# quantumgizmos/bp_osd

Hardware: AMD Instinct MI355X
Metric: syndromes decoded/sec (whole node) + logical error rate, HGP [[1922,50]] p=0.05 (higher is better)
Workload: dtype f64; 1 GPU; h1922_ms_cs7: [[1922,50]] HGP (31x31 circulant 1+x^2+x^5) hz 961x1922, min-sum BP variable scaling, max_iter=1922, osd_cs order 7, iid bit-flip q=0.05; per_gpu_batch=131072, global_batch=131072, bp_variant=0, pipelined_steps=2, hw_queues=4, batches=2 distinct seeded batches alternate over the timed steps

## Files before the change

### bp_osd_amd/_lib.py

```python
from __future__ import annotations

import ctypes as C
import os

_HERE = os.path.dirname(os.path.abspath(__file__))
LIB_PATH = os.environ.get("BPOSD_LIB") or os.path.join(_HERE, "libbposd_mi355x.so")

BPOSD_OK = 0
BPOSD_ERR_INVALID = -1
BPOSD_ERR_UNSUPPORTED = -2
BPOSD_ERR_HIP = -3
BPOSD_ERR_NO_DEVICE = -4

EXPORTED_SYMBOLS = (
    "bposd_device_count",
    "bposd_version",
    "bposd_create",
    "bposd_update_channel_probs",
    "bposd_decode_batch",
    "bposd_decode_batch_packed",
    "bposd_decode_batch_async",
    "bposd_decode_batch_packed_async",
    "bposd_decode_batch_device",
    "bposd_decode_batch_device_packed",
# ... 9 lines not shown
    "bposd_host_alloc",
    "bposd_host_free",
    "bposd_last_timing",
    "bposd_info",
    "bposd_posterior_llr",
    "bposd_set_bp_variant",
    "bposd_set_osd_variant",
    "bposd_last_osd_kernel",
    "bposd_mc_create",
    "bposd_mc_run",
    "bposd_mc_fetch",
    "bposd_mc_device_bytes",
    "bposd_mc_last_error",
    "bposd_mc_destroy",
    "bposd_last_error",
    "bposd_destroy",
)

DEBUG_SYMBOLS = (
    "bposd_layout_info",
    "bposd_bp_kernel_info",
    "bposd_debug_local_layout",
    "bposd_debug_local_keys",
    "bposd_debug_class_layout",
    "bposd_debug_last_instance",
)


class BposdConfig(C.Structure):
    _fields_ = [
        ("device", C.c_int32),
        ("bp_method", C.c_int32),
        ("ms_scaling_factor", C.c_double),
        ("max_iter", C.c_int32),
        ("osd_method", C.c_int32),
        ("osd_order", C.c_int32),
        ("sort_tie_policy", C.c_int32),
        ("weight_fn", C.c_int32),
        ("schedule", C.c_int32),
        ("ps_clip", C.c_double),
        ("osd_e_bit_order", C.c_int32),
        ("ps_math_form", C.c_int32),
    ]


class BposdMcConfig(C.Structure):
# ... 61 lines not shown
    lib.bposd_lane_timing.restype = C.c_int
    lib.bposd_host_alloc.argtypes = [C.c_size_t]
    lib.bposd_host_alloc.restype = vp
    lib.bposd_host_free.argtypes = [vp]
    lib.bposd_host_free.restype = None
    lib.bposd_last_timing.argtypes = [vp, C.POINTER(C.c_double), C.POINTER(C.c_double),
                                      C.POINTER(C.c_int64), C.POINTER(C.c_int64)]
    lib.bposd_last_timing.restype = C.c_int
    lib.bposd_info.argtypes = [vp, C.POINTER(C.c_int32), C.POINTER(C.c_int32), C.POINTER(C.c_int32),
                               C.POINTER(C.c_int32)]
    lib.bposd_info.restype = C.c_int
    lib.bposd_layout_info.argtypes = [vp, C.POINTER(C.c_int64), C.POINTER(C.c_int64), C.POINTER(C.c_int64)]
    lib.bposd_layout_info.restype = C.c_int
    lib.bposd_pack_rows_device_lane.argtypes = [vp, C.c_int32, vp, C.c_int64, C.c_int32, vp]
    lib.bposd_pack_rows_device_lane.restype = C.c_int
    lib.bposd_posterior_llr.argtypes = [vp, vp, C.c_int64, vp, vp, vp, vp]
    lib.bposd_posterior_llr.restype = C.c_int
    lib.bposd_bp_kernel_info.argtypes = [vp, C.POINTER(C.c_int32), vp]
    lib.bposd_bp_kernel_info.restype = C.c_int
    lib.bposd_debug_local_layout.argtypes = [vp, vp, C.c_int32, C.c_int32, vp]
    lib.bposd_debug_local_layout.restype = C.c_int
    lib.bposd_debug_local_keys.argtypes = [vp, vp, C.c_int32, C.c_int32, vp, vp, vp]
    lib.bposd_debug_local_keys.restype = C.c_int
    lib.bposd_debug_class_layout.argtypes = [vp, vp, C.c_int32, C.c_int32, vp, vp, vp, vp, vp, vp]
    lib.bposd_debug_class_layout.restype = C.c_int
    lib.bposd_debug_last_instance.argtypes = [vp, vp, vp]
    lib.bposd_debug_last_instance.restype = C.c_int
    lib.bposd_set_osd_variant.argtypes = [vp, C.c_int32]
    lib.bposd_set_osd_variant.restype = C.c_int
    lib.bposd_last_osd_kernel.argtypes = [vp]
    lib.bposd_last_osd_kernel.restype = C.c_int
    lib.bposd_set_bp_variant.argtypes = [vp, C.c_int32]
    lib.bposd_set_bp_variant.restype = C.c_int
    lib.bposd_last_error.argtypes = [vp]
    lib.bposd_last_error.restype = C.c_char_p
    lib.bposd_destroy.argtypes = [vp]
    lib.bposd_destroy.restype = None
    lib.bposd_mc_create.argtypes = [C.POINTER(BposdMcConfig), vp, vp, vp, vp, C.c_int32, vp, vp, C.c_int32, C.c_int32, vp, vp, C.c_int32,
                                    vp, vp, vp, vp, C.POINTER(vp)]
    lib.bposd_mc_create.restype = C.c_int
    lib.bposd_mc_run.argtypes = [vp, C.c_uint64, C.c_int64, C.POINTER(C.c_int64)]
    lib.bposd_mc_run.restype = C.c_int
    lib.bposd_mc_fetch.argtypes = [vp, C.c_int32, vp, C.c_size_t]
    lib.bposd_mc_fetch.restype = C.c_int
    lib.bposd_mc_device_bytes.argtypes = [vp]
    lib.bposd_mc_device_bytes.restype = C.c_int64
# ... 27 lines not shown
```

### bp_osd_amd/csrc/bp_local_kernel.hip.h

```cpp
#pragma once
#include <hip/hip_runtime.h>
#include <stdint.h>

#include "bp_kernel.hip.h"
#include "local_keys.h"

#ifndef BPOSD_BPL_SIGN_ON_MAG
#define BPOSD_BPL_SIGN_ON_MAG 0
#endif
namespace bposd {

struct BpLocalParams {
    int m, n;
    long long B;
    int max_iter;
    double ms_scaling;
    int osd_enabled;
    int mp;
    const uint8_t* __restrict__ synd;
    const double* __restrict__ llr0;
    const uint8_t* __restrict__ sel;
    const double* __restrict__ llr0_alt;
    const int* __restrict__ pos_chk;
    const int* __restrict__ pos_bit;
// ... 58 lines not shown

__device__ __forceinline__ int bpl_table_load(const int* base, unsigned int lane_off, unsigned int const_off) {
    asm volatile("" : "+v"(lane_off));
    return *(const int*)((const char*)base + (lane_off + const_off));
}

static_assert(__is_trivially_copyable(BpLocalParams) && alignof(BpLocalParams) <= 8, "BpLocalParams is copied into the kernarg segment as it is");
typedef const __attribute__((address_space(4))) BpLocalParams* bpl_args_ptr;
__device__ __forceinline__ bpl_args_ptr bpl_args() {
    bpl_args_ptr a = (bpl_args_ptr)__builtin_amdgcn_kernarg_segment_ptr();
    asm volatile("" : "+s"(a));
    return a;
}

template <int V>
struct bpl_int {
    static constexpr int value = V;
};

__host__ __device__ constexpr bool bpl_specialised(int cpt, int mpt, int minw, bool early) {
    return !early && ((cpt == 1 && mpt == 1024 && minw == 8) || (cpt == 2 && mpt == 1024 && (minw == 8 || minw == 6)) || (cpt == 2 && mpt == 2048 && minw == 4));
}

template <int CPT, int MPT, int MINW, bool EARLY, bool UPRIOR, bool PACKED = false>
__global__ __launch_bounds__(MPT / CPT, MINW) void bp_local_kernel(const BpLocalParams P) {
    extern __shared__ __attribute__((aligned(16))) unsigned char smem[];
    const int m = P.m, n = P.n;
#ifdef BPOSD_DEBUG
    if (blockIdx.x == 0 && threadIdx.x == 0 && (bpl_args()->m != P.m || bpl_args()->counters != P.counters)) __builtin_trap();
#endif
    constexpr int NT = MPT / CPT;
    constexpr int MP = MPT;
    const int tid = threadIdx.x;
    const int lane = tid & 63;
    const int wave = __builtin_amdgcn_readfirstlane(tid >> 6);
    constexpr int NB = 2 * CPT;

    double* msg_plain = reinterpret_cast<double*>(smem);
    msg_ptr msg = (msg_ptr)msg_plain;
    unsigned int* diffw = reinterpret_cast<unsigned int*>(msg_plain + (size_t)4 * MP + 2);
    int* sh = reinterpret_cast<int*>(diffw + (MP / 32 + 2));
    const unsigned int diffw_base = (unsigned int)(uintptr_t)(__attribute__((address_space(3))) unsigned char*)diffw;

    typedef __attribute__((address_space(3))) unsigned char* lds_bytes;
    const unsigned int msg_base = (unsigned int)(uintptr_t)(lds_bytes)smem;
    unsigned int alo[NB], ahi[NB];
    int dl[NB];
    unsigned int dlpack = 0u;
    double l0[UPRIOR ? 1 : NB];
    if (UPRIOR) {
// ... 6 lines not shown
#pragma unroll
    for (int j = 0; j < CPT; ++j) {
        const int p = tid + j * NT;
#pragma unroll
        for (int b = 0; b < 2; ++b) {
            const int r = 2 * j + b;
            if (!UPRIOR) {
                const int bit = BPL_BIT(r);
                l0[r] = bit >= 0 ? bpl_args()->llr0[bit] : 1.0;
            }
            alo[r] = msg_base + 8u * (unsigned int)bpl_args()->pos_alo[b * MP + p];
            ahi[r] = msg_base + 8u * (unsigned int)bpl_args()->pos_ahi[b * MP + p];
            dl[r] = __builtin_amdgcn_readfirstlane(bpl_args()->grp_dl[b * (MP >> 6) + (p >> 6)]);
            dlpack |= (unsigned int)bpl_args()->pos_dl[b * MP + p] << (2 * r);
        }
    }

    int gkey[CPT];
#pragma unroll
    for (int j = 0; j < CPT; ++j) gkey[j] = bposd_local_keys::group_key(dl[2 * j], dl[2 * j + 1]);
    int wkey = gkey[0];
#pragma unroll
    for (int j = 1; j < CPT; ++j) wkey = (gkey[j] == wkey) ? wkey : -1;
    constexpr bool SPEC = bpl_specialised(CPT, MPT, MINW, EARLY);

    const int want_llr_s = __builtin_amdgcn_readfirstlane(bpl_args()->out_llr != nullptr ? 1 : 0);
    auto want_llr = [&]() -> bool {
        int w = want_llr_s;
        asm volatile("" : "+s"(w));
        return w != 0;
    };
    for (;;) {
        if (tid == 0) {
            int zero = 0;
            asm volatile("" : "+v"(zero));
            sh[0] = zero;
            sh[1] = zero;
            sh[2] = atomicAdd(&bpl_args()->counters[0], 1);
        }
        __syncthreads();
        const long long s = __builtin_amdgcn_readfirstlane(sh[2]);
        if (s >= P.B) {
            if (s == P.B && tid == 0 && bpl_args()->tail_flag) *(volatile int*)bpl_args()->tail_flag = 1;
            break;
        }

// ... 157 lines not shown
                        unsigned int pa = alo[r], pb = ahi[r];
                        asm volatile("" : "+v"(pa), "+v"(pb));
                        const int ca = (int)((pa - msg_base) >> 3) & (MP - 1), cb = (int)((pb - msg_base) >> 3) & (MP - 1);
                        const int co = tid + (r >> 1) * NT;
                        atomicXor(&diffw[ca >> 5], 1u << (ca & 31));
                        atomicXor(&diffw[cb >> 5], 1u << (cb & 31));
                        atomicXor(&diffw[co >> 5], 1u << (co & 31));
                    }
                };
                auto group_step = [&](const int j, auto gk_c) __attribute__((always_inline)) {
                    constexpr int GK = decltype(gk_c)::value;
                    bit_step(2 * j, bpl_int<bposd_local_keys::key_dl(GK, 0)>{});
                    bit_step(2 * j + 1, bpl_int<bposd_local_keys::key_dl(GK, 1)>{});
                };
#pragma unroll
                for (int j = 0; j < CPT; ++j) {
                    if ((2 * j) % BATCH == 0) {
#pragma unroll
                        for (int q = 2 * j; q < 2 * j + BATCH; ++q) {
                            X[q] = *BPL_AT(alo[q]);
                            Y[q] = *BPL_AT(ahi[q]);
                        }
                    }
                    if constexpr (KEY >= 0) group_step(j, bpl_int<KEY>{});
                    else {
                        switch (gkey[j]) {
                            case 0: group_step(j, bpl_int<0>{}); break;
                            case 1: group_step(j, bpl_int<1>{}); break;
                            case 2: group_step(j, bpl_int<2>{}); break;
                            case 5: group_step(j, bpl_int<5>{}); break;
                            case 6: group_step(j, bpl_int<6>{}); break;
                            case 10: group_step(j, bpl_int<10>{}); break;
                            default: group_step(j, bpl_int<bposd_local_keys::kMixedKey>{}); break;
                        }
                    }
                }
                __syncthreads();
            }
            return 0;
        };
        if (!conv) {
            int done = 0;
            int it_llr = 1;
            if (!want_llr()) {
                int wk = wkey;
                asm volatile("" : "+s"(wk));
                if constexpr (SPEC) {
                    switch (wk) {
                        case 0: done = iterate(bpl_int<0>{}, bpl_int<0>{}, 1); break;
                        case 1: done = iterate(bpl_int<1>{}, bpl_int<0>{}, 1); break;
                        case 2: done = iterate(bpl_int<2>{}, bpl_int<0>{}, 1); break;
                        case 5: done = iterate(bpl_int<5>{}, bpl_int<0>{}, 1); break;
                        case 6: done = iterate(bpl_int<6>{}, bpl_int<0>{}, 1); break;
                        case 10: done = iterate(bpl_int<10>{}, bpl_int<0>{}, 1); break;
                        case bposd_local_keys::kMixedKey: done = iterate(bpl_int<bposd_local_keys::kMixedKey>{}, bpl_int<0>{}, 1); break;
                        default: done = iterate(bpl_int<-1>{}, bpl_int<0>{}, 1); break;
                    }
                } else done = iterate(bpl_int<-1>{}, bpl_int<0>{}, 1);
                asm volatile("" : "+s"(done));
                it_llr = bpl_args()->max_iter;
                it_llr = it_llr > 1 ? it_llr : 1;
            }
            if (!done) iterate(bpl_int<-1>{}, bpl_int<1>{}, it_llr);
        }

        const bool to_osd = (!conv) && bpl_args()->osd_enabled;
        if (tid == 0) {
            if (to_osd) {
                const int slot = atomicAdd(&bpl_args()->counters[1], 1);
                bpl_args()->osd_list[slot] = (int)s;
                sh[3] = slot;
            }
            if (bpl_args()->out_conv) bpl_args()->out_conv[s] = conv ? 1 : 0;
            if (bpl_args()->out_iters) bpl_args()->out_iters[s] = it_done;
            if (it_done) atomicAdd(bpl_args()->iter_total, (unsigned long long)it_done);
        }
        __syncthreads();
        const int slot = to_osd ? sh[3] : 0;
        constexpr bool packed = PACKED;
// ... 32 lines not shown
```

### bp_osd_amd/csrc/bposd_capi.hip

```cpp
#include "../../include/bposd_mi355x.h"

#include <hip/hip_runtime.h>

#include <algorithm>
#include <cmath>
#include <cstdarg>
#include <cstdio>
#include <cstdlib>
#include <climits>
#include <cstring>
#include <string>
#include <tuple>
#include <functional>
#include <map>
#include <chrono>
#include <mutex>
#include <thread>
#include <vector>

#include "internal.h"
#include <array>
#include <vector>
#include <algorithm>
#include "local_layout.h"
// ... 282 lines not shown
    h->tab_dc = DC;
    h->tab_dv = DV;
    h->tab_mp = MP;
    h->tab_np = NP;
    return 0;
}
int build_tables_local(bposd_handle* h) {
    using namespace local_layout;
    h->local_ok = false;
    const int m = h->m, n = h->n;
    if (!(h->regular && h->dc_max == 6 && h->dv_max == 3 && n == 2 * m)) return 0;
    const int MP = m <= 1024 ? 1024 : 2048;
    if (m > MP) return 0;
    Graph g;
    Layout best;
    if (!local_layout_host(h->rp, h->ci, m, n, MP, g, best)) return 0;
    if (getenv("BPOSD_DEBUG_OCC"))
        fprintf(stderr, "[bposd] local-edge layout: bit pass %lld read cycles (floor %d) + %lld write cycles (floor %d), %d mixed pairs, %d uniform positions\n",
                best.passes, 4 * (MP / 32), best.wcycles, 6 * 4 * (MP / 64), best.mixed, best.nfull);
    h->local_passes = best.passes;
    h->local_wcycles = best.wcycles;

    const std::vector<int>&owner = best.owner, &load = best.load, &pos_of = best.pos_of, &pos_chk = best.pos_chk;
    const std::vector<int> grp_dl = group_dl_table(g, best);
    auto slot_of = [&](int c, int i) {
        int k = 0;
        for (int e = h->rp[c]; e < h->rp[c + 1]; ++e) {
            const int j = h->ci[e];
            if (owner[j] == c) continue;
            if (j == i) return k * MP + pos_of[c];
            ++k;
        }
        return -1;
    };
    std::vector<int> pos_bit(2 * (size_t)MP, -1), pos_alo(2 * (size_t)MP, 0), pos_ahi(2 * (size_t)MP, 0), pos_dl(2 * (size_t)MP, 0);
    for (int p = 0; p < MP; ++p)
        for (int b = 0; b < 2; ++b) {
            pos_alo[(size_t)b * MP + p] = (2 * b) * MP + p;
            pos_ahi[(size_t)b * MP + p] = (2 * b + 1) * MP + p;
        }
    for (int c = 0; c < m; ++c) {
        const int p = pos_of[c];
        for (int b = 0; b < 2; ++b) {
            const int i = load[2 * c + b];
            int o[2];
            g.others(i, c, o);
            const int sx = slot_of(o[0], i), sy = slot_of(o[1], i);
// ... 576 lines not shown

int bposd_bp_kernel_info(bposd_handle* h, int32_t* kernel, int64_t* lds_model) {
    if (!h) return BPOSD_ERR_INVALID;
    if (kernel) *kernel = h->last_bp_kernel;
    if (lds_model) {
        for (int k = 0; k < 4; ++k) lds_model[k] = 0;
        if (h->last_bp_kernel == BPOSD_BP_KERNEL_LOCAL) {
            lds_model[0] = h->local_passes; lds_model[1] = 4 * (h->local_mp / 32);
            lds_model[2] = h->local_wcycles; lds_model[3] = 6 * 4 * (h->local_mp / 64);
        } else if (h->last_bp_kernel == BPOSD_BP_KERNEL_CLASS) {
            lds_model[0] = h->class_read_cycles; lds_model[1] = h->class_read_floor;
            lds_model[2] = h->class_write_cycles; lds_model[3] = h->class_write_floor;
        } else if (h->last_bp_kernel == BPOSD_BP_KERNEL_LARGE) {
            lds_model[0] = h->large_form;
        }
    }
    return BPOSD_OK;
}

int bposd_debug_last_instance(bposd_handle* h, int32_t bp[6], int32_t osd[6]) {
    if (!h) return BPOSD_ERR_INVALID;
    if (bp) std::copy(h->last_bp_inst, h->last_bp_inst + 6, bp);
    if (osd) std::copy(h->last_osd_inst, h->last_osd_inst + 6, osd);
    return BPOSD_OK;
}

int bposd_synchronize(bposd_handle* h) {
    if (!h) return BPOSD_ERR_INVALID;
    DeviceGuard dev_guard(h->device);
    HIP_TRY(h, dev_guard.err);
    return sync_all_lanes(h);
}

static int decode_device_impl(bposd_handle* h, const uint8_t* d_synd, int64_t B, const uint8_t* d_sel,
                              uint8_t* d_osdw, uint8_t* d_osd0, uint8_t* d_bp, uint8_t* d_conv,
                              int32_t* d_iters, double* d_llr, int lane = -1, int rec_idx = 0, bool lean = false) {
    if (!h) return BPOSD_ERR_INVALID;
    if (B < 0 || B > 0x7fffffffLL) return fail(h, BPOSD_ERR_INVALID, "batch size %lld out of range", (long long)B);
    if (B == 0) return BPOSD_OK;
    if (!d_synd || !d_osdw) return fail(h, BPOSD_ERR_INVALID, "syndromes and osdw buffers are required");
    DeviceGuard dev_guard(h->device);
    HIP_TRY(h, dev_guard.err);
    if (lane < 0) {
        lane = h->next_lane;
        h->next_lane = (h->next_lane + 1) % h->nlanes;
        h->last_lane = lane;
// ... 681 lines not shown
        if (rp[c + 1] - rp[c] != 6) return BPOSD_ERR_UNSUPPORTED;
    std::vector<int> deg(n, 0);
    for (int e : ci) {
        if (e < 0 || e >= n) return BPOSD_ERR_INVALID;
        deg[e]++;
    }
    for (int i = 0; i < n; ++i)
        if (deg[i] != 3) return BPOSD_ERR_UNSUPPORTED;
    local_layout::Graph g;
    local_layout::Layout best;
    if (!local_layout_host(rp, ci, m, n, MP, g, best, false)) return BPOSD_ERR_UNSUPPORTED;
    local_layout::LdsCost t = local_layout::lds_cost(g, best);
    info[0] = t.read_cycles; info[1] = t.write_cycles; info[2] = t.mixed;
    if (local_layout::pair_groups(g, best) < 0) return BPOSD_ERR_UNSUPPORTED;
    t = local_layout::lds_cost(g, best);
    info[3] = t.read_cycles; info[4] = t.write_cycles; info[5] = t.mixed;
    info[6] = MP; info[7] = best.generic_waves;
    const std::vector<int> keys = local_layout::group_keys(g, best);
    for (int gq = 0; gq < MP / 64; ++gq) group_key[gq] = keys[gq];
    for (int p = 0; p < MP; ++p) pos_chk[p] = best.pos_chk[p];
    return BPOSD_OK;
}

int bposd_debug_class_layout(const int32_t* indptr, const int32_t* indices, int32_t m, int32_t n, int32_t* pos_chk, int32_t* pos_bit,
                             int32_t* bit_slot, int32_t* grp_deg, int32_t* grp_cdeg, int64_t* info) {
    if (!indptr || !indices || !info || m < 1 || n < 1) return BPOSD_ERR_INVALID;
    std::vector<int> rp(indptr, indptr + m + 1), ci(indices, indices + indptr[m]);
    for (int e : ci)
        if (e < 0 || e >= n) return BPOSD_ERR_INVALID;
    const ClassShape* shp = class_shape_for(rp, ci, m, n);
    if (!shp || m > 1024) return BPOSD_ERR_UNSUPPORTED;
    class_layout::Tables T;
    bool ok = false;
    for (int mp : {256, 512, 1024}) {
        if (m > mp) continue;
        if (class_layout::build(rp, ci, m, n, shp->dclo, shp->dc, shp->dvlo, shp->dvhi, kClassVPT, mp, mp, class_layout_iters(), T)) { ok = true; break; }
    }
    if (!ok) return BPOSD_ERR_UNSUPPORTED;
    info[0] = shp->dc; info[1] = shp->dvlo; info[2] = shp->dvhi; info[3] = kClassVPT; info[4] = T.MP; info[5] = T.NT;
    info[6] = T.read_cycles; info[7] = T.read_floor; info[8] = T.write_cycles; info[9] = T.write_floor; info[10] = shp->dclo;
    if (pos_chk) std::copy(T.pos_chk.begin(), T.pos_chk.end(), pos_chk);
    if (pos_bit) std::copy(T.pos_bit.begin(), T.pos_bit.end(), pos_bit);
    if (bit_slot) std::copy(T.bit_slot.begin(), T.bit_slot.end(), bit_slot);
    if (grp_deg) std::copy(T.grp_deg.begin(), T.grp_deg.end(), grp_deg);
    if (grp_cdeg) std::copy(T.grp_cdeg.begin(), T.grp_cdeg.end(), grp_cdeg);
    return BPOSD_OK;
// ... 14 lines not shown
```

### bp_osd_amd/csrc/internal.h

```cpp
#pragma once
#include "../../include/bposd_mi355x.h"
#include "../../include/bposd_mi355x_debug.h"

#include <hip/hip_runtime.h>

#include <algorithm>
#include <cstdio>
#include <cstdlib>
#include <string>
#include <vector>

#include "bp_kernel.hip.h"
#include "osd_kernel.hip.h"

struct DevBuf {
    void* p = nullptr;
    size_t bytes = 0;
};

constexpr int BPOSD_LANES = 4;
constexpr int BPOSD_MAX_CHUNKS = 16;

struct Lane {
    hipStream_t stream = nullptr;
// ... 51 lines not shown
    int dc_max = 0, dv_max = 0;
    bool regular = false;
    bool local_ok = false;
    int local_mp = 0;
    long long local_passes = 0;
    long long local_wcycles = 0;
    int *d_lpos_chk = nullptr, *d_lpos_bit = nullptr, *d_lpos_alo = nullptr, *d_lpos_ahi = nullptr, *d_lgrp_dl = nullptr, *d_lpos_dl = nullptr;
    bool bp_any = false;
    bool class_ok = false;
    int class_dclo = 0, class_dc = 0, class_dvlo = 0, class_dvhi = 0, class_mp = 0, class_nt = 0;
    long class_read_cycles = 0, class_write_cycles = 0, class_read_floor = 0, class_write_floor = 0;
    int *d_cpos_chk = nullptr, *d_cpos_bit = nullptr, *d_cbit_slot = nullptr, *d_cgrp_deg = nullptr, *d_cgrp_cdeg = nullptr;
    bool large = false;
    bool bp_hbm = false;
    int max_iter = 0;
    int rank = 0, kprime = 0, ncand = 0;
    bool probs_uniform = true;
    int bp_variant = 0;
    int last_bp_kernel = -1;
    int osd_variant = 0;
    int last_osd_kernel = -1;
    int32_t last_bp_inst[6] = {-1, 0, 0, 0, 0, 0};
    int32_t last_osd_inst[6] = {-1, 0, 0, 0, 0, 0};
    std::vector<int> rp, ci;
    std::vector<double> probs;
    int *d_rp = nullptr, *d_ci = nullptr;
    int *d_chk_deg = nullptr, *d_var_deg = nullptr, *d_var_pos = nullptr, *d_pos_bit = nullptr, *d_var_ck = nullptr;
    int large_form = 0;
    int tab_np = 0;
    long layout_cost = 0, layout_cost_natural = 0, layout_cost_ideal = 0;
    double* d_llr0 = nullptr;
    double* d_cost = nullptr;
    double *d_llr0_alt = nullptr, *d_cost_alt = nullptr;
    bool fp_weights = false;
    int *d_cp = nullptr, *d_ce = nullptr, *d_erow = nullptr, *d_lvl_ptr = nullptr, *d_lvl_bits = nullptr;
    int nlevels = 0;
    int tab_dc = 0, tab_dv = 0, tab_mp = 0;
    bool have_timing = false;
    long long batch_hint = 0;
    bool async_pending = false;
    hipStream_t osd_now = nullptr;
    uint8_t *cmp_osd0 = nullptr, *cmp_osdw = nullptr;
    bool bp_only = false;
    bool lane_alt = false;
    bool packed_now = false;
    bool tail_gate = false;
// ... 53 lines not shown
```

### bp_osd_amd/csrc/launch_bp_local.hip

```cpp
#include "internal.h"

#include "bp_local_kernel.hip.h"

using namespace bposd;
using namespace bposd_host;

namespace bposd_host {
template <int CPT, int MP, int MINW, bool EARLY, bool UPRIOR, bool PACKED>
static int launch_bp_local_tp(bposd_handle* h, const BpLocalParams& L);

template <int CPT, int MP, int MINW, bool EARLY, bool UPRIOR = false>
static int launch_bp_local_t(bposd_handle* h, const BpLocalParams& L) {
    constexpr bool has_packed = !EARLY && ((CPT == 1 && MP == 1024 && MINW == 8) || (CPT == 2 && MP == 1024 && (MINW == 8 || MINW == 6)) || MP == 2048);
    if constexpr (has_packed) {
        if (L.packed_io) return launch_bp_local_tp<CPT, MP, MINW, EARLY, UPRIOR, true>(h, L);
    } else {
        if (L.packed_io) return fail(h, BPOSD_ERR_UNSUPPORTED, "this BP kernel variant has no packed-I/O form");
    }
    return launch_bp_local_tp<CPT, MP, MINW, EARLY, UPRIOR, false>(h, L);
}

template <int CPT, int MP, int MINW, bool EARLY, bool UPRIOR, bool PACKED>
static int launch_bp_local_tp(bposd_handle* h, const BpLocalParams& L) {
    auto k = bp_local_kernel<CPT, MP, MINW, EARLY, UPRIOR, PACKED>;
    const int nt = MP / CPT;
    const size_t lds = bp_local_lds_bytes(L.mp);
    { int rc_lds = set_max_lds(h, (const void*)k, lds); if (rc_lds) return rc_lds; }
    int wg_per_cu = 1;
    { int rc_occ = cached_occupancy(h, (const void*)k, nt, lds, &wg_per_cu); if (rc_occ) return rc_occ; }
    if (getenv("BPOSD_DEBUG_OCC")) fprintf(stderr, "[bposd] local-edge BP kernel: %d threads, %zu B LDS, %d workgroups per CU\n", nt, lds, wg_per_cu);
    wg_per_cu = std::max(1, std::min(wg_per_cu, 8));
    long long grid = std::min<long long>(L.B, (long long)h->num_cu * wg_per_cu);
    if (grid < 1) grid = 1;
    int rc = ensure_lanes(h, &Lane::bpl_llr, sizeof(double) * (size_t)grid * h->n);
    if (rc) return rc;
    BpLocalParams Lq = L;
    Lq.llr_tmp = (double*)h->cur->bpl_llr.p;
    note_instance(h->last_bp_inst, BPOSD_BP_KERNEL_LOCAL, CPT, MP, MINW, EARLY, PACKED);
    hipLaunchKernelGGL(k, dim3((unsigned)grid), dim3(nt), lds, h->cur->stream, Lq);
    HIP_TRY(h, hipGetLastError());
    return 0;
}

int launch_bp_local(bposd_handle* h, const BpParams& P) {
    BpLocalParams L{};
    L.m = P.m; L.n = P.n; L.B = P.B; L.max_iter = P.max_iter; L.ms_scaling = P.ms_scaling; L.osd_enabled = P.osd_enabled;
    L.mp = h->local_mp;
    L.synd = P.synd; L.llr0 = P.llr0; L.sel = P.sel; L.llr0_alt = P.llr0_alt;
    L.pos_chk = h->d_lpos_chk; L.pos_bit = h->d_lpos_bit; L.pos_alo = h->d_lpos_alo; L.pos_ahi = h->d_lpos_ahi;
    L.grp_dl = h->d_lgrp_dl; L.pos_dl = h->d_lpos_dl;
    L.out_bp = P.out_bp; L.out_osd0 = P.out_osd0; L.out_osdw = P.out_osdw; L.out_conv = P.out_conv; L.out_iters = P.out_iters;
    L.out_llr = P.out_llr; L.llr_ws = P.llr_ws; L.osd_list = P.osd_list; L.counters = P.counters; L.iter_total = P.iter_total; L.tail_flag = P.tail_flag; L.packed_io = P.packed_io;
    if (h->local_mp == 2048) return launch_bp_local_t<2, 2048, 4, false>(h, L);
    if (h->bp_variant == 17) return launch_bp_local_t<2, 1024, 8, false>(h, L);
    if (h->bp_variant == 18) return launch_bp_local_t<1, 1024, 8, false>(h, L);
    if (h->bp_variant == 19) return launch_bp_local_t<4, 1024, 4, true>(h, L);
    if (h->bp_variant == 20) return launch_bp_local_t<2, 1024, 6, true>(h, L);
    if (h->bp_variant == 21) return launch_bp_local_t<4, 1024, 3, true>(h, L);
    const bool uprior = h->probs_uniform && !L.sel && h->probs[0] > 0.0 && h->probs[0] < 0.5;
    const long long work = h->batch_hint > 0 ? h->batch_hint : L.B;
    const bool small_call = h->bp_variant == 0 && work <= 40000;
    if (small_call) return uprior ? launch_bp_local_t<1, 1024, 8, false, true>(h, L) : launch_bp_local_t<1, 1024, 8, false>(h, L);
    if ((h->bp_variant == 22 || h->bp_variant == 0) && uprior) return launch_bp_local_t<2, 1024, 8, false, true>(h, L);
    if (h->bp_variant == 23 && uprior) return launch_bp_local_t<2, 1024, 6, true, true>(h, L);
    if (h->bp_variant == 24 && uprior) return launch_bp_local_t<2, 1024, 6, false, true>(h, L);
    if (h->bp_variant == 25 && uprior) return launch_bp_local_t<2, 1024, 8, true, true>(h, L);
    if (h->bp_variant == 26 && uprior) return launch_bp_local_t<1, 1024, 8, false, true>(h, L);
    return launch_bp_local_t<2, 1024, 6, false>(h, L);
}
}
```

### bp_osd_amd/csrc/local_keys.h

```cpp
#pragma once

namespace bposd_local_keys {

constexpr int kMixedKey = 15;
constexpr int kNumKeys = 7;
constexpr int kKeys[kNumKeys] = {0, 1, 2, 5, 6, 10, 15};

constexpr int group_key(int dl0, int dl1) { return (dl0 >= 0 && dl0 <= dl1 && dl1 < 3) ? 4 * dl0 + dl1 : kMixedKey; }
constexpr int key_dl(int key, int slot) { return key == kMixedKey ? 3 : (slot == 0 ? key / 4 : key % 4); }

}
```

### bp_osd_amd/csrc/local_layout.h

```cpp
#pragma once
#include <algorithm>
#include <cmath>
#include <cstdio>
#include <cstdlib>
#include <functional>
#include <thread>
#include <vector>

#include "local_keys.h"

namespace local_layout {

struct Layout {
    std::vector<int> owner;
    std::vector<int> load;
    std::vector<int> pos_of;
    std::vector<int> pos_chk;
    int nfull = 0;
    double cost = 1e30;
    long long passes = 0;
    long long wcycles = 0;
    int mixed = 0;
    int generic_waves = 0;
};

struct Graph {
    int m, n, MP;
// ... 311 lines not shown
    const int G = g.MP / 64, W = G / 2;
    std::vector<int> key(G);
    for (int gq = 0; gq < G; ++gq) {
        const int c0 = group_code(g, L, gq, 0), c1 = group_code(g, L, gq, 1);
        key[gq] = c0 < 0 ? -1 : bposd_local_keys::group_key(c0, c1);
    }
    std::vector<std::pair<int, int>> pairs;
    std::vector<int> singles, empties;
    std::vector<char> used(G, 0);
    for (int gq = 0; gq < G; ++gq) {
        if (used[gq]) continue;
        if (key[gq] < 0) { empties.push_back(gq); used[gq] = 1; continue; }
        int mate = -1;
        for (int q = gq + 1; q < G && mate < 0; ++q)
            if (!used[q] && key[q] == key[gq]) mate = q;
        used[gq] = 1;
        if (mate < 0) { singles.push_back(gq); continue; }
        used[mate] = 1;
        pairs.push_back({gq, mate});
    }
    int generic = 0;
    size_t e = 0, s1 = 0;
    for (; s1 < singles.size() && e < empties.size(); ++s1, ++e) pairs.push_back({std::min(singles[s1], empties[e]), std::max(singles[s1], empties[e])});
    for (; s1 + 1 < singles.size(); s1 += 2, ++generic) pairs.push_back({singles[s1], singles[s1 + 1]});
    for (; e + 1 < empties.size(); e += 2) pairs.push_back({empties[e], empties[e + 1]});
    if ((int)pairs.size() != W) return -1;
    std::sort(pairs.begin(), pairs.end());
    std::vector<int> new_of(G);
    for (int w = 0; w < W; ++w) { new_of[pairs[w].first] = w; new_of[pairs[w].second] = w + W; }
    std::vector<int> pos_chk(g.MP, -1);
    for (int p = 0; p < g.MP; ++p) {
        const int c = L.pos_chk[p];
        const int q = 64 * new_of[p >> 6] + (p & 63);
        pos_chk[q] = c;
        if (c >= 0) L.pos_of[c] = q;
    }
    L.pos_chk = pos_chk;
    L.generic_waves = generic;
    return generic;
}

}

inline bool local_layout_host(const std::vector<int>& rp, const std::vector<int>& ci, int m, int n, int MP,
                              local_layout::Graph& g, local_layout::Layout& best, bool pair = true) {
    using namespace local_layout;
    g.m = m; g.n = n; g.MP = MP;
    g.cols.assign(3 * (size_t)n, 0);
    {
        std::vector<int> fill(n, 0);
        for (int c = 0; c < m; ++c)
            for (int e = rp[c]; e < rp[c + 1]; ++e) {
                const int i = ci[e];
                g.cols[3 * (size_t)i + fill[i]++] = c;
            }
    }
    const std::vector<int>& cols = g.cols;
    std::vector<Layout> cands;
    {
        Layout L;
        L.owner.assign(n, -1);
        L.load.assign(2 * (size_t)m, -1);
// ... 62 lines not shown
                L.load = slot;
                cands.push_back(L);
            }
    }
    {
        const size_t n0 = cands.size();
        for (size_t k = 0; k < n0; ++k)
            for (int sideways = 0; sideways < 2; ++sideways) {
                Layout R = cands[k];
                if (rebalance_classes(g, R, MP / 64, 100000, sideways != 0)) { cands.push_back(R); break; }
            }
    }
    {
        double mixw = 5.0;
        if (const char* e = getenv("BPOSD_MIXW")) mixw = atof(e);
        auto total = [&](const Layout& L) { return L.cost - 5.0 * L.mixed + mixw * L.mixed; };
        std::vector<std::pair<double, size_t>> rank;
        for (size_t k = 0; k < cands.size(); ++k) {
            class_sorted(g, cands[k]);
            search(g, cands[k], true, 0);
            rank.push_back({total(cands[k]), k});
        }
        std::sort(rank.begin(), rank.end());
        const size_t nfinish = std::min(rank.size(), getenv("BPOSD_LAYOUT_ALL") ? rank.size() : (size_t)3);
        const int iters = getenv("BPOSD_LAYOUT_ITERS") ? atoi(getenv("BPOSD_LAYOUT_ITERS")) : 400000;
        std::vector<Layout> fin(nfinish);
        std::vector<std::thread> th;
        for (size_t q = 0; q < nfinish; ++q) {
            fin[q] = cands[rank[q].second];
            th.emplace_back([&g, &fin, q, iters]() { search(g, fin[q], true, iters); });
        }
        for (auto& t : th) t.join();
        for (size_t q = 0; q < nfinish; ++q) {
            if (getenv("BPOSD_DEBUG_OCC"))
                fprintf(stderr, "[bposd] candidate %zu: %lld read + %lld write cycles, %d mixed pairs\n", rank[q].second, fin[q].passes,
                        fin[q].wcycles, fin[q].mixed);
            if (q == 0 || total(fin[q]) < total(best)) best = fin[q];
        }
    }
    if (pair) {
        if (pair_groups(g, best) < 0) return false;
        const LdsCost t = lds_cost(g, best);
        best.passes = t.read_cycles;
        best.wcycles = t.write_cycles;
        best.mixed = t.mixed;
        if (getenv("BPOSD_DEBUG_OCC")) fprintf(stderr, "[bposd] wave pairing: %d generic wave(s) of %d\n", best.generic_waves, MP / 128);
// ... 5 lines not shown
```

### bp_osd_amd/decoder.py

```python
from __future__ import annotations

import ctypes as C

import sys

import numpy as np
import scipy.sparse as sp

from . import _lib

__all__ = ["BpOsdDecoder", "bposd_decoder"]

_BP_METHODS = {
    "product_sum": 0, "prod_sum": 0, "ps": 0, "0": 0,
    "minimum_sum": 1, "min_sum": 1, "ms": 1, "1": 1,
}
_BP_NAMES = {0: "product_sum", 1: "minimum_sum"}
_OSD_METHODS = {
    "osd_off": 0, "off": 0,
    "osd_0": 1, "osd0": 1, "0": 1, "osd_zero": 1,
    "osd_e": 2, "osde": 2, "e": 2, "exhaustive": 2,
    "osd_cs": 3, "osdcs": 3, "cs": 3, "combination_sweep": 3,
}
_OSD_NAMES = {0: "osd_off", 1: "osd_0", 2: "osd_e", 3: "osd_cs"}
# ... 476 lines not shown
    def set_osd_variant(self, variant: int):
        _lib.check(self._lib, self._h, self._lib.bposd_set_osd_variant(self._h, int(variant)))

    def last_osd_kernel(self):
        return self.OSD_KERNEL_NAMES.get(self._lib.bposd_last_osd_kernel(self._h), "none")

    _BP_INSTANCE_ARITY = {0: 4, 1: 4, 2: 4, 3: 3, 4: 0, 5: 0}
    _OSD_INSTANCE_ARITY = {1: 1, 2: 2, 3: 1, 4: 4}

    def last_instance(self):
        bp = np.zeros(6, dtype=np.int32)
        osd = np.zeros(6, dtype=np.int32)
        _lib.check(self._lib, self._h, self._lib.bposd_debug_last_instance(self._h, bp.ctypes.data, osd.ctypes.data))

        def entry(v, names, arity):
            code = int(v[0])
            if code not in names:
                return ("none", (), False)
            return (names[code], tuple(int(x) for x in v[1:1 + arity[code]]), bool(v[5]))

        return {"bp": entry(bp, self.BP_KERNEL_NAMES, self._BP_INSTANCE_ARITY),
                "osd": entry(osd, self.OSD_KERNEL_NAMES, self._OSD_INSTANCE_ARITY)}

    def set_bp_variant(self, variant: int):
        _lib.check(self._lib, self._h, self._lib.bposd_set_bp_variant(self._h, int(variant)))

    def update_channel_probs(self, channel_probs):
        p = np.ascontiguousarray(channel_probs, dtype=np.float64)
        if p.shape != (self.n,):
            raise ValueError(f"The error channel vector must have length {self.n}, not {p.shape}")
        rc = self._lib.bposd_update_channel_probs(self._h, p.ctypes.data)
        _lib.check(self._lib, self._h, rc)
        if self._single is not None and self._single[5] is None and 5 not in self._single_cache and self._llr_probs is None:
            self._llr_probs = self._probs
        self._probs = p.copy()

    @property
    def osdw_decoding(self):
        return self._attr(0)

    @property
    def osd0_decoding(self):
        return self._attr(1)

    @property
    def bp_decoding(self):
# ... 76 lines not shown
```

### include/bposd_mi355x_debug.h

```cpp
#ifndef BPOSD_MI355X_DEBUG_H
#define BPOSD_MI355X_DEBUG_H

#include "bposd_mi355x.h"

#ifdef __cplusplus
extern "C" {
#endif
#pragma GCC visibility push(default)

int bposd_layout_info(bposd_handle *h, int64_t *natural_cycles, int64_t *chosen_cycles, int64_t *ideal_cycles);

#define BPOSD_BP_KERNEL_LDS 0
#define BPOSD_BP_KERNEL_LOCAL 1
#define BPOSD_BP_KERNEL_CLASS 2
#define BPOSD_BP_KERNEL_LARGE 3
#define BPOSD_BP_KERNEL_SERIAL 4
#define BPOSD_BP_KERNEL_ANYDEG 5
int bposd_bp_kernel_info(bposd_handle *h, int32_t *kernel, int64_t *lds_model);

int bposd_debug_last_instance(bposd_handle *h, int32_t bp[6], int32_t osd[6]);

int bposd_debug_local_layout(const int32_t *csr_indptr, const int32_t *csr_indices, int32_t m, int32_t n, int64_t *out);

int bposd_debug_local_keys(const int32_t *csr_indptr, const int32_t *csr_indices, int32_t m, int32_t n, int32_t *group_key,
                           int32_t *pos_chk, int64_t *info);

int bposd_debug_class_layout(const int32_t *csr_indptr, const int32_t *csr_indices, int32_t m, int32_t n, int32_t *pos_chk,
                             int32_t *pos_bit, int32_t *bit_slot, int32_t *grp_deg, int32_t *grp_cdeg, int64_t *info);

#pragma GCC visibility pop
#ifdef __cplusplus
}
#endif
#endif
```

Before: 5.623 million syndromes/s.

## Add pair-key specialised BP wave bodies for mixed waves in local kernel

```diff
diff --git a/bp_osd_amd/_lib.py b/bp_osd_amd/_lib.py
--- a/bp_osd_amd/_lib.py
+++ b/bp_osd_amd/_lib.py
@@ -55,6 +55,8 @@
     "bposd_bp_kernel_info",
     "bposd_debug_local_layout",
     "bposd_debug_local_keys",
+    "bposd_debug_local_waves",
+    "bposd_debug_last_pair_key",
     "bposd_debug_class_layout",
     "bposd_debug_last_instance",
 )
@@ -162,6 +164,10 @@
     lib.bposd_debug_local_layout.restype = C.c_int
     lib.bposd_debug_local_keys.argtypes = [vp, vp, C.c_int32, C.c_int32, vp, vp, vp]
     lib.bposd_debug_local_keys.restype = C.c_int
+    lib.bposd_debug_local_waves.argtypes = [vp, vp, C.c_int32, C.c_int32, vp, vp]
+    lib.bposd_debug_local_waves.restype = C.c_int
+    lib.bposd_debug_last_pair_key.argtypes = [vp, C.POINTER(C.c_int32)]
+    lib.bposd_debug_last_pair_key.restype = C.c_int
     lib.bposd_debug_class_layout.argtypes = [vp, vp, C.c_int32, C.c_int32, vp, vp, vp, vp, vp, vp]
     lib.bposd_debug_class_layout.restype = C.c_int
     lib.bposd_debug_last_instance.argtypes = [vp, vp, vp]
diff --git a/bp_osd_amd/csrc/bp_local_kernel.hip.h b/bp_osd_amd/csrc/bp_local_kernel.hip.h
--- a/bp_osd_amd/csrc/bp_local_kernel.hip.h
+++ b/bp_osd_amd/csrc/bp_local_kernel.hip.h
@@ -104,10 +104,10 @@
     return !early && ((cpt == 1 && mpt == 1024 && minw == 8) || (cpt == 2 && mpt == 1024 && (minw == 8 || minw == 6)) || (cpt == 2 && mpt == 2048 && minw == 4));
 }
 
-template <int CPT, int MPT, int MINW, bool EARLY, bool UPRIOR, bool PACKED = false>
+template <int CPT, int MPT, int MINW, bool EARLY, bool UPRIOR, bool PACKED = false, int PAIRKEY = -1>
 __global__ __launch_bounds__(MPT / CPT, MINW) void bp_local_kernel(const BpLocalParams P) {
     extern __shared__ __attribute__((aligned(16))) unsigned char smem[];
-    const int m = P.m, n = P.n;
+    const int m = PAIRKEY >= 0 ? bpl_args()->m : P.m, n = PAIRKEY >= 0 ? bpl_args()->n : P.n;
 #ifdef BPOSD_DEBUG
     if (blockIdx.x == 0 && threadIdx.x == 0 && (bpl_args()->m != P.m || bpl_args()->counters != P.counters)) __builtin_trap();
 #endif
@@ -160,6 +160,11 @@
     int wkey = gkey[0];
 #pragma unroll
     for (int j = 1; j < CPT; ++j) wkey = (gkey[j] == wkey) ? wkey : -1;
+    constexpr int PKEY = bposd_local_keys::pair_key(PAIRKEY);
+    static_assert(PKEY < 0 || (CPT == 2 && bpl_specialised(CPT, MPT, MINW, EARLY)), "a pair body is for two groups per wave");
+    if constexpr (PKEY >= 0) {
+        if (gkey[0] == PAIRKEY && gkey[CPT - 1] == bposd_local_keys::kMixedKey) wkey = PKEY;
+    }
     constexpr bool SPEC = bpl_specialised(CPT, MPT, MINW, EARLY);
 
     const int want_llr_s = __builtin_amdgcn_readfirstlane(bpl_args()->out_llr != nullptr ? 1 : 0);
@@ -363,8 +368,10 @@
                             Y[q] = *BPL_AT(ahi[q]);
                         }
                     }
-                    if constexpr (KEY >= 0) group_step(j, bpl_int<KEY>{});
-                    else {
+                    if constexpr (KEY >= 0) {
+                        if (j == 0) group_step(j, bpl_int<bposd_local_keys::body_group_key(KEY, 0)>{});
+                        else group_step(j, bpl_int<bposd_local_keys::body_group_key(KEY, 1)>{});
+                    } else {
                         switch (gkey[j]) {
                             case 0: group_step(j, bpl_int<0>{}); break;
                             case 1: group_step(j, bpl_int<1>{}); break;
@@ -395,7 +402,10 @@
                         case 6: done = iterate(bpl_int<6>{}, bpl_int<0>{}, 1); break;
                         case 10: done = iterate(bpl_int<10>{}, bpl_int<0>{}, 1); break;
                         case bposd_local_keys::kMixedKey: done = iterate(bpl_int<bposd_local_keys::kMixedKey>{}, bpl_int<0>{}, 1); break;
-                        default: done = iterate(bpl_int<-1>{}, bpl_int<0>{}, 1); break;
+                        default:
+                            if (PKEY >= 0 && wk == PKEY) done = iterate(bpl_int<(PKEY >= 0 ? PKEY : -1)>{}, bpl_int<0>{}, 1);
+                            else done = iterate(bpl_int<-1>{}, bpl_int<0>{}, 1);
+                            break;
                     }
                 } else done = iterate(bpl_int<-1>{}, bpl_int<0>{}, 1);
                 asm volatile("" : "+s"(done));
diff --git a/bp_osd_amd/csrc/bposd_capi.hip b/bp_osd_amd/csrc/bposd_capi.hip
--- a/bp_osd_amd/csrc/bposd_capi.hip
+++ b/bp_osd_amd/csrc/bposd_capi.hip
@@ -328,7 +328,14 @@
     h->local_wcycles = best.wcycles;
 
     const std::vector<int>&owner = best.owner, &load = best.load, &pos_of = best.pos_of, &pos_chk = best.pos_chk;
-    const std::vector<int> grp_dl = group_dl_table(g, best);
+    const WavePlan plan = wave_plan(g, best, pair_mode());
+    const std::vector<int>& grp_dl = plan.grp_dl;
+    h->local_pair_key = plan.pair_key;
+    if (getenv("BPOSD_DEBUG_OCC")) {
+        fprintf(stderr, "[bposd] wave bodies (-1 generic):");
+        for (int b : plan.body) fprintf(stderr, " %d", b);
+        fprintf(stderr, "; instance PAIRKEY %d, %d generic wave(s)\n", plan.pair_key, plan.generic);
+    }
     auto slot_of = [&](int c, int i) {
         int k = 0;
         for (int e = h->rp[c]; e < h->rp[c + 1]; ++e) {
@@ -951,6 +958,12 @@
     if (!h) return BPOSD_ERR_INVALID;
     if (bp) std::copy(h->last_bp_inst, h->last_bp_inst + 6, bp);
     if (osd) std::copy(h->last_osd_inst, h->last_osd_inst + 6, osd);
+    return BPOSD_OK;
+}
+
+int bposd_debug_last_pair_key(bposd_handle* h, int32_t* pair_key) {
+    if (!h || !pair_key) return BPOSD_ERR_INVALID;
+    *pair_key = h->last_bp_inst[0] == BPOSD_BP_KERNEL_LOCAL ? h->last_bp_pair_key : -1;
     return BPOSD_OK;
 }
 
@@ -1678,6 +1691,30 @@
     return BPOSD_OK;
 }
 
+int bposd_debug_local_waves(const int32_t* indptr, const int32_t* indices, int32_t m, int32_t n, int32_t* wave_body, int64_t* info) {
+    if (!indptr || !indices || !wave_body || !info || n != 2 * m) return BPOSD_ERR_INVALID;
+    std::vector<int> rp(indptr, indptr + m + 1), ci(indices, indices + indptr[m]);
+    const int MP = m <= 1024 ? 1024 : 2048;
+    if (m > MP) return BPOSD_ERR_UNSUPPORTED;
+    for (int c = 0; c < m; ++c)
+        if (rp[c + 1] - rp[c] != 6) return BPOSD_ERR_UNSUPPORTED;
+    std::vector<int> deg(n, 0);
+    for (int e : ci) {
+        if (e < 0 || e >= n) return BPOSD_ERR_INVALID;
+        deg[e]++;
+    }
+    for (int i = 0; i < n; ++i)
+        if (deg[i] != 3) return BPOSD_ERR_UNSUPPORTED;
+    local_layout::Graph g;
+    local_layout::Layout best;
+    if (!local_layout_host(rp, ci, m, n, MP, g, best)) return BPOSD_ERR_UNSUPPORTED;
+    const local_layout::PairMode mode = local_layout::pair_mode();
+    const local_layout::WavePlan plan = local_layout::wave_plan(g, best, mode);
+    for (int w = 0; w < MP / 128; ++w) wave_body[w] = plan.body[w];
+    info[0] = MP; info[1] = plan.pair_key; info[2] = plan.generic; info[3] = (int)mode;
+    return BPOSD_OK;
+}
+
 int bposd_debug_class_layout(const int32_t* indptr, const int32_t* indices, int32_t m, int32_t n, int32_t* pos_chk, int32_t* pos_bit,
                              int32_t* bit_slot, int32_t* grp_deg, int32_t* grp_cdeg, int64_t* info) {
     if (!indptr || !indices || !info || m < 1 || n < 1) return BPOSD_ERR_INVALID;
diff --git a/bp_osd_amd/csrc/internal.h b/bp_osd_amd/csrc/internal.h
--- a/bp_osd_amd/csrc/internal.h
+++ b/bp_osd_amd/csrc/internal.h
@@ -97,6 +97,8 @@
     int last_osd_kernel = -1;
     int32_t last_bp_inst[6] = {-1, 0, 0, 0, 0, 0};
     int32_t last_osd_inst[6] = {-1, 0, 0, 0, 0, 0};
+    int local_pair_key = -1;
+    int last_bp_pair_key = -1;
     std::vector<int> rp, ci;
     std::vector<double> probs;
     int *d_rp = nullptr, *d_ci = nullptr;
diff --git a/bp_osd_amd/csrc/launch_bp_local.h b/bp_osd_amd/csrc/launch_bp_local.h
--- /dev/null
+++ b/bp_osd_amd/csrc/launch_bp_local.h
@@ -0,0 +1,36 @@
+#pragma once
+#include "internal.h"
+
+#include "bp_local_kernel.hip.h"
+
+namespace bposd_host {
+
+template <int CPT, int MP, int MINW, bool EARLY, bool UPRIOR, bool PACKED, int PAIRKEY = -1>
+static int launch_bp_local_tp(bposd_handle* h, const bposd::BpLocalParams& L) {
+    using namespace bposd;
+    auto k = bp_local_kernel<CPT, MP, MINW, EARLY, UPRIOR, PACKED, PAIRKEY>;
+    const int nt = MP / CPT;
+    const size_t lds = bp_local_lds_bytes(L.mp);
+    { int rc_lds = set_max_lds(h, (const void*)k, lds); if (rc_lds) return rc_lds; }
+    int wg_per_cu = 1;
+    { int rc_occ = cached_occupancy(h, (const void*)k, nt, lds, &wg_per_cu); if (rc_occ) return rc_occ; }
+    if (getenv("BPOSD_DEBUG_OCC")) fprintf(stderr, "[bposd] local-edge BP kernel: %d threads, %zu B LDS, %d workgroups per CU, PAIRKEY %d\n", nt, lds, wg_per_cu, PAIRKEY);
+    wg_per_cu = std::max(1, std::min(wg_per_cu, 8));
+    long long grid = std::min<long long>(L.B, (long long)h->num_cu * wg_per_cu);
+    if (grid < 1) grid = 1;
+    int rc = ensure_lanes(h, &Lane::bpl_llr, sizeof(double) * (size_t)grid * h->n);
+    if (rc) return rc;
+    BpLocalParams Lq = L;
+    Lq.llr_tmp = (double*)h->cur->bpl_llr.p;
+    note_instance(h->last_bp_inst, BPOSD_BP_KERNEL_LOCAL, CPT, MP, MINW, EARLY, PACKED);
+    h->last_bp_pair_key = PAIRKEY;
+    hipLaunchKernelGGL(k, dim3((unsigned)grid), dim3(nt), lds, h->cur->stream, Lq);
+    HIP_TRY(h, hipGetLastError());
+    return 0;
+}
+
+enum BplPairShape { kBplPair1024x8U = 0, kBplPair1024x6 = 1, kBplPair2048x4 = 2 };
+template <int KEY>
+int launch_bp_local_pair(bposd_handle* h, const bposd::BpLocalParams& L, int shape);
+
+}
diff --git a/bp_osd_amd/csrc/launch_bp_local.hip b/bp_osd_amd/csrc/launch_bp_local.hip
--- a/bp_osd_amd/csrc/launch_bp_local.hip
+++ b/bp_osd_amd/csrc/launch_bp_local.hip
@@ -1,14 +1,9 @@
-#include "internal.h"
-
-#include "bp_local_kernel.hip.h"
+#include "launch_bp_local.h"
 
 using namespace bposd;
 using namespace bposd_host;
 
 namespace bposd_host {
-template <int CPT, int MP, int MINW, bool EARLY, bool UPRIOR, bool PACKED>
-static int launch_bp_local_tp(bposd_handle* h, const BpLocalParams& L);
-
 template <int CPT, int MP, int MINW, bool EARLY, bool UPRIOR = false>
 static int launch_bp_local_t(bposd_handle* h, const BpLocalParams& L) {
     constexpr bool has_packed = !EARLY && ((CPT == 1 && MP == 1024 && MINW == 8) || (CPT == 2 && MP == 1024 && (MINW == 8 || MINW == 6)) || MP == 2048);
@@ -20,26 +15,16 @@
     return launch_bp_local_tp<CPT, MP, MINW, EARLY, UPRIOR, false>(h, L);
 }
 
-template <int CPT, int MP, int MINW, bool EARLY, bool UPRIOR, bool PACKED>
-static int launch_bp_local_tp(bposd_handle* h, const BpLocalParams& L) {
-    auto k = bp_local_kernel<CPT, MP, MINW, EARLY, UPRIOR, PACKED>;
-    const int nt = MP / CPT;
-    const size_t lds = bp_local_lds_bytes(L.mp);
-    { int rc_lds = set_max_lds(h, (const void*)k, lds); if (rc_lds) return rc_lds; }
-    int wg_per_cu = 1;
-    { int rc_occ = cached_occupancy(h, (const void*)k, nt, lds, &wg_per_cu); if (rc_occ) return rc_occ; }
-    if (getenv("BPOSD_DEBUG_OCC")) fprintf(stderr, "[bposd] local-edge BP kernel: %d threads, %zu B LDS, %d workgroups per CU\n", nt, lds, wg_per_cu);
-    wg_per_cu = std::max(1, std::min(wg_per_cu, 8));
-    long long grid = std::min<long long>(L.B, (long long)h->num_cu * wg_per_cu);
-    if (grid < 1) grid = 1;
-    int rc = ensure_lanes(h, &Lane::bpl_llr, sizeof(double) * (size_t)grid * h->n);
-    if (rc) return rc;
-    BpLocalParams Lq = L;
-    Lq.llr_tmp = (double*)h->cur->bpl_llr.p;
-    note_instance(h->last_bp_inst, BPOSD_BP_KERNEL_LOCAL, CPT, MP, MINW, EARLY, PACKED);
-    hipLaunchKernelGGL(k, dim3((unsigned)grid), dim3(nt), lds, h->cur->stream, Lq);
-    HIP_TRY(h, hipGetLastError());
-    return 0;
+static int launch_bp_local_pair_any(bposd_handle* h, const BpLocalParams& L, int shape) {
+    switch (h->local_pair_key) {
+        case 0: return launch_bp_local_pair<0>(h, L, shape);
+        case 1: return launch_bp_local_pair<1>(h, L, shape);
+        case 2: return launch_bp_local_pair<2>(h, L, shape);
+        case 5: return launch_bp_local_pair<5>(h, L, shape);
+        case 6: return launch_bp_local_pair<6>(h, L, shape);
+        case 10: return launch_bp_local_pair<10>(h, L, shape);
+    }
+    return fail(h, BPOSD_ERR_UNSUPPORTED, "no bp_local_kernel instance with a pair body for key %d", h->local_pair_key);
 }
 
 int launch_bp_local(bposd_handle* h, const BpParams& P) {
@@ -51,7 +36,8 @@
     L.grp_dl = h->d_lgrp_dl; L.pos_dl = h->d_lpos_dl;
     L.out_bp = P.out_bp; L.out_osd0 = P.out_osd0; L.out_osdw = P.out_osdw; L.out_conv = P.out_conv; L.out_iters = P.out_iters;
     L.out_llr = P.out_llr; L.llr_ws = P.llr_ws; L.osd_list = P.osd_list; L.counters = P.counters; L.iter_total = P.iter_total; L.tail_flag = P.tail_flag; L.packed_io = P.packed_io;
-    if (h->local_mp == 2048) return launch_bp_local_t<2, 2048, 4, false>(h, L);
+    const bool pair = h->bp_variant == 0 && h->local_pair_key >= 0;
+    if (h->local_mp == 2048) return pair ? launch_bp_local_pair_any(h, L, kBplPair2048x4) : launch_bp_local_t<2, 2048, 4, false>(h, L);
     if (h->bp_variant == 17) return launch_bp_local_t<2, 1024, 8, false>(h, L);
     if (h->bp_variant == 18) return launch_bp_local_t<1, 1024, 8, false>(h, L);
     if (h->bp_variant == 19) return launch_bp_local_t<4, 1024, 4, true>(h, L);
@@ -61,6 +47,7 @@
     const long long work = h->batch_hint > 0 ? h->batch_hint : L.B;
     const bool small_call = h->bp_variant == 0 && work <= 40000;
     if (small_call) return uprior ? launch_bp_local_t<1, 1024, 8, false, true>(h, L) : launch_bp_local_t<1, 1024, 8, false>(h, L);
+    if (pair) return launch_bp_local_pair_any(h, L, uprior ? kBplPair1024x8U : kBplPair1024x6);
     if ((h->bp_variant == 22 || h->bp_variant == 0) && uprior) return launch_bp_local_t<2, 1024, 8, false, true>(h, L);
     if (h->bp_variant == 23 && uprior) return launch_bp_local_t<2, 1024, 6, true, true>(h, L);
     if (h->bp_variant == 24 && uprior) return launch_bp_local_t<2, 1024, 6, false, true>(h, L);
diff --git a/bp_osd_amd/csrc/launch_bp_local_pair.inc.h b/bp_osd_amd/csrc/launch_bp_local_pair.inc.h
--- /dev/null
+++ b/bp_osd_amd/csrc/launch_bp_local_pair.inc.h
@@ -0,0 +1,18 @@
+#include "launch_bp_local.h"
+
+namespace bposd_host {
+template <>
+int launch_bp_local_pair<BPL_PAIRKEY>(bposd_handle* h, const bposd::BpLocalParams& L, int shape) {
+    constexpr int K = BPL_PAIRKEY;
+    static_assert(bposd_local_keys::pair_key(K) >= 0, "a uniform key of local_keys.h");
+    switch (shape) {
+        case kBplPair1024x8U:
+            return L.packed_io ? launch_bp_local_tp<2, 1024, 8, false, true, true, K>(h, L) : launch_bp_local_tp<2, 1024, 8, false, true, false, K>(h, L);
+        case kBplPair1024x6:
+            return L.packed_io ? launch_bp_local_tp<2, 1024, 6, false, false, true, K>(h, L) : launch_bp_local_tp<2, 1024, 6, false, false, false, K>(h, L);
+        case kBplPair2048x4:
+            return L.packed_io ? launch_bp_local_tp<2, 2048, 4, false, false, true, K>(h, L) : launch_bp_local_tp<2, 2048, 4, false, false, false, K>(h, L);
+    }
+    return fail(h, BPOSD_ERR_UNSUPPORTED, "no bp_local_kernel instance with a pair body for shape %d", shape);
+}
+}
diff --git a/bp_osd_amd/csrc/launch_bp_local_pair_k0.hip b/bp_osd_amd/csrc/launch_bp_local_pair_k0.hip
--- /dev/null
+++ b/bp_osd_amd/csrc/launch_bp_local_pair_k0.hip
@@ -0,0 +1,2 @@
+#define BPL_PAIRKEY 0
+#include "launch_bp_local_pair.inc.h"
diff --git a/bp_osd_amd/csrc/launch_bp_local_pair_k1.hip b/bp_osd_amd/csrc/launch_bp_local_pair_k1.hip
--- /dev/null
+++ b/bp_osd_amd/csrc/launch_bp_local_pair_k1.hip
@@ -0,0 +1,2 @@
+#define BPL_PAIRKEY 1
+#include "launch_bp_local_pair.inc.h"
diff --git a/bp_osd_amd/csrc/launch_bp_local_pair_k10.hip b/bp_osd_amd/csrc/launch_bp_local_pair_k10.hip
--- /dev/null
+++ b/bp_osd_amd/csrc/launch_bp_local_pair_k10.hip
@@ -0,0 +1,2 @@
+#define BPL_PAIRKEY 10
+#include "launch_bp_local_pair.inc.h"
diff --git a/bp_osd_amd/csrc/launch_bp_local_pair_k2.hip b/bp_osd_amd/csrc/launch_bp_local_pair_k2.hip
--- /dev/null
+++ b/bp_osd_amd/csrc/launch_bp_local_pair_k2.hip
@@ -0,0 +1,2 @@
+#define BPL_PAIRKEY 2
+#include "launch_bp_local_pair.inc.h"
diff --git a/bp_osd_amd/csrc/launch_bp_local_pair_k5.hip b/bp_osd_amd/csrc/launch_bp_local_pair_k5.hip
--- /dev/null
+++ b/bp_osd_amd/csrc/launch_bp_local_pair_k5.hip
@@ -0,0 +1,2 @@
+#define BPL_PAIRKEY 5
+#include "launch_bp_local_pair.inc.h"
diff --git a/bp_osd_amd/csrc/launch_bp_local_pair_k6.hip b/bp_osd_amd/csrc/launch_bp_local_pair_k6.hip
--- /dev/null
+++ b/bp_osd_amd/csrc/launch_bp_local_pair_k6.hip
@@ -0,0 +1,2 @@
+#define BPL_PAIRKEY 6
+#include "launch_bp_local_pair.inc.h"
diff --git a/bp_osd_amd/csrc/local_keys.h b/bp_osd_amd/csrc/local_keys.h
--- a/bp_osd_amd/csrc/local_keys.h
+++ b/bp_osd_amd/csrc/local_keys.h
@@ -9,4 +9,11 @@
 constexpr int group_key(int dl0, int dl1) { return (dl0 >= 0 && dl0 <= dl1 && dl1 < 3) ? 4 * dl0 + dl1 : kMixedKey; }
 constexpr int key_dl(int key, int slot) { return key == kMixedKey ? 3 : (slot == 0 ? key / 4 : key % 4); }
 
+constexpr int kNumPairKeys = 6;
+constexpr int kPairKeys[kNumPairKeys] = {32, 33, 34, 37, 38, 42};
+
+constexpr int pair_key(int k) { return (k >= 0 && k < kMixedKey) ? 32 + k : -1; }
+constexpr bool is_pair_key(int key) { return key >= 32; }
+constexpr int body_group_key(int key, int j) { return is_pair_key(key) ? (j == 0 ? key - 32 : kMixedKey) : key; }
+
 }
diff --git a/bp_osd_amd/csrc/local_layout.h b/bp_osd_amd/csrc/local_layout.h
--- a/bp_osd_amd/csrc/local_layout.h
+++ b/bp_osd_amd/csrc/local_layout.h
@@ -3,6 +3,7 @@
 #include <cmath>
 #include <cstdio>
 #include <cstdlib>
+#include <cstring>
 #include <functional>
 #include <thread>
 #include <vector>
@@ -360,6 +361,8 @@
     int generic = 0;
     size_t e = 0, s1 = 0;
     for (; s1 < singles.size() && e < empties.size(); ++s1, ++e) pairs.push_back({std::min(singles[s1], empties[e]), std::max(singles[s1], empties[e])});
+    if (singles.size() - s1 >= 2)
+        std::stable_sort(singles.begin() + s1, singles.end(), [&](int a, int b) { return (key[a] == bposd_local_keys::kMixedKey) < (key[b] == bposd_local_keys::kMixedKey); });
     for (; s1 + 1 < singles.size(); s1 += 2, ++generic) pairs.push_back({singles[s1], singles[s1 + 1]});
     for (; e + 1 < empties.size(); e += 2) pairs.push_back({empties[e], empties[e + 1]});
     if ((int)pairs.size() != W) return -1;
@@ -376,6 +379,50 @@
     L.pos_chk = pos_chk;
     L.generic_waves = generic;
     return generic;
+}
+
+enum PairMode { kPairGeneric = 0, kPairDemote = 1, kPairBody = 2 };
+inline PairMode pair_mode() {
+    if (const char* e = getenv("BPOSD_PAIR_MODE")) {
+        if (!strcmp(e, "generic")) return kPairGeneric;
+        if (!strcmp(e, "demote")) return kPairDemote;
+        if (!strcmp(e, "body")) return kPairBody;
+    }
+    return kPairBody;
+}
+
+struct WavePlan {
+    std::vector<int> grp_dl;
+    std::vector<int> body;
+    int pair_key = -1;
+    int generic = 0;
+};
+
+inline WavePlan wave_plan(const Graph& g, const Layout& L, PairMode mode) {
+    using namespace bposd_local_keys;
+    const int G = g.MP / 64, W = G / 2;
+    WavePlan P;
+    P.grp_dl = group_dl_table(g, L);
+    P.body.assign(W, -1);
+    std::vector<int> key(G);
+    for (int gq = 0; gq < G; ++gq) key[gq] = group_key(P.grp_dl[gq], P.grp_dl[(size_t)G + gq]);
+    if (mode == kPairBody) {
+        int count[kMixedKey] = {0};
+        for (int w = 0; w < W; ++w)
+            if (key[w] != kMixedKey && key[w + W] == kMixedKey) count[key[w]]++;
+        for (int k = 0; k < kMixedKey; ++k)
+            if (count[k] > (P.pair_key < 0 ? 0 : count[P.pair_key])) P.pair_key = k;
+    }
+    for (int w = 0; w < W; ++w) {
+        const int a = key[w], b = key[w + W];
+        if (a == b) P.body[w] = a;
+        else if (mode == kPairDemote && (a == kMixedKey || b == kMixedKey)) {
+            for (int s = 0; s < 2; ++s) P.grp_dl[(size_t)s * G + w] = P.grp_dl[(size_t)s * G + w + W] = 3;
+            P.body[w] = kMixedKey;
+        } else if (mode == kPairBody && a == P.pair_key && b == kMixedKey) P.body[w] = pair_key(a);
+        P.generic += P.body[w] < 0;
+    }
+    return P;
 }
 
 }
@@ -484,6 +531,10 @@
             rank.push_back({total(cands[k]), k});
         }
         std::sort(rank.begin(), rank.end());
+        if (const char* e = getenv("BPOSD_LAYOUT_PIN")) {
+            const size_t k = (size_t)atoi(e);
+            if (k < cands.size()) rank.assign(1, {total(cands[k]), k});
+        }
         const size_t nfinish = std::min(rank.size(), getenv("BPOSD_LAYOUT_ALL") ? rank.size() : (size_t)3);
         const int iters = getenv("BPOSD_LAYOUT_ITERS") ? atoi(getenv("BPOSD_LAYOUT_ITERS")) : 400000;
         std::vector<Layout> fin(nfinish);
diff --git a/bp_osd_amd/decoder.py b/bp_osd_amd/decoder.py
--- a/bp_osd_amd/decoder.py
+++ b/bp_osd_amd/decoder.py
@@ -522,6 +522,11 @@
         return {"bp": entry(bp, self.BP_KERNEL_NAMES, self._BP_INSTANCE_ARITY),
                 "osd": entry(osd, self.OSD_KERNEL_NAMES, self._OSD_INSTANCE_ARITY)}
 
+    def last_pair_key(self) -> int:
+        k = C.c_int32(-1)
+        _lib.check(self._lib, self._h, self._lib.bposd_debug_last_pair_key(self._h, C.byref(k)))
+        return int(k.value)
+
     def set_bp_variant(self, variant: int):
         _lib.check(self._lib, self._h, self._lib.bposd_set_bp_variant(self._h, int(variant)))
 
diff --git a/include/bposd_mi355x_debug.h b/include/bposd_mi355x_debug.h
--- a/include/bposd_mi355x_debug.h
+++ b/include/bposd_mi355x_debug.h
@@ -25,6 +25,11 @@
 int bposd_debug_local_keys(const int32_t *csr_indptr, const int32_t *csr_indices, int32_t m, int32_t n, int32_t *group_key,
                            int32_t *pos_chk, int64_t *info);
 
+int bposd_debug_local_waves(const int32_t *csr_indptr, const int32_t *csr_indices, int32_t m, int32_t n, int32_t *wave_body,
+                            int64_t *info);
+
+int bposd_debug_last_pair_key(bposd_handle *h, int32_t *pair_key);
+
 int bposd_debug_class_layout(const int32_t *csr_indptr, const int32_t *csr_indices, int32_t m, int32_t n, int32_t *pos_chk,
                              int32_t *pos_bit, int32_t *bit_slot, int32_t *grp_deg, int32_t *grp_cdeg, int64_t *info);
 
```

Result: faster. 5.729 million syndromes/s, median of 6 (+1.9%).
